# craston/object_detection_cib

Hardware: AMD Instinct MI355X
Metric: images/sec YOLOv5s 640px train (higher is better)
Workload: dtype bf16; 1 GPU; yv5s coco-zipf-like synthetic, 640px, bf16 storage/fp32 accumulate, batch 64/GPU, fwd+assign+loss+bwd+SGD, targets 4-30 boxes/img; global_batch=64, parallelism=dp1, launch=hipGraph replay, collectives=none, launcher=none, attempt=0

## Files before the change

### object_detection_cib_amd/csrc/conv_igemm.hip

```cpp
#include "kodhip_common.h"
#include <stdlib.h>
#include <type_traits>

extern "C" const char* kodhip_last_error(void);

namespace {

enum { MODE_RAW = 0, MODE_PLAIN = 1, MODE_HEAD = 2, MODE_PLAIN_BN = 3, MODE_FUSED = 4, MODE_FUSED_ACT = 5 };

constexpr bool mode_is_fused(int mode) { return mode == MODE_FUSED || mode == MODE_FUSED_ACT; }

constexpr int MAX_SEG = 3;

struct ConvArgs {
  const bf16_t* x;
  const bf16_t* w;
  bf16_t* y;
  float* stats;
  const float* bias;
  float* head_out;
  int B, Hs, Ws, ldx, xcoff, Cin;
  int cin_step;
  int Ho, Wo, M;
  int N, K, Kp;
  int KH, KW;
  int mul_h, mul_w, add_h, add_w, tap_sign, sh_shift, sw_shift;
  int ldy, ycoff, accumulate;
  float* y32;
  int f32_mode;
  int out_mul, out_off_y, out_off_x, out_H, out_W;
  int d2s_C;
  int d2s_skip;
  int head_A, head_P, head_nc;
  uint32_t magic_hp;
  uint32_t magic_cin, magic_kw;
  int tiles_m, tiles_n, groups_m, stats_slots;
  float rcp_hwo, rcp_wo;
  uint32_t x_bytes, w_bytes;
  const bf16_t* x2;
  const bf16_t* w2;
  int nk1;
  int wide_px;
  int pointwise;
  int nseg, slot_base, slot_used;
  int seg_begin[MAX_SEG], seg_end[MAX_SEG], seg_ldr[MAX_SEG], seg_C[MAX_SEG];
  const bf16_t* seg_raw[MAX_SEG];
  const float* seg_aff[MAX_SEG];
  float* seg_part[MAX_SEG];
  const float* scale;
  const float* shift;
  const bf16_t* residual;
  int ldr, rcoff;
  int act;
  float slope;
};

template <int ACT>
__device__ __forceinline__ bf16x4 fused_quad(const f32x16& acc, int g, const f32x4& sc, const f32x4& sh, float slope) {
  bf16x4 v;
#pragma unroll
  for (int e = 0; e < 4; ++e) v[e] = (bf16_t)kod_act<ACT>(__builtin_fmaf(acc[g * 4 + e], sc[e], sh[e]), slope);
  return v;
}

__device__ __forceinline__ void fast_divmod(int n, int d, float rcp, int& q, int& r) {
  q = (int)((float)n * rcp);
  r = n - q * d;
  while (r < 0) { --q; r += d; }
  while (r >= d) { ++q; r -= d; }
}

constexpr int BK = 32;

template <int N>
__device__ __forceinline__ void wait_vm_imm() { asm volatile("s_waitcnt vmcnt(%0)" ::"n"(N) : "memory"); }

template <int BM, int BN, int WAVES_M, int WAVES_N, int MODE, bool FAST, bool ROW3 = false, bool F32ACC = false, bool STEM = false>
__device__ __forceinline__ void conv_igemm_body(const ConvArgs& a, const int bid) {
  constexpr int NT = 64 * WAVES_M * WAVES_N;
  constexpr int NW = NT / 64;
  static_assert(FAST || (BM == 128 && NT == 256), "register-staged path is written for 128-row tiles / 4 waves");
  constexpr int LDS_ROW = FAST ? BK : BK + 8;
  constexpr int WM = BM / WAVES_M;
  constexpr int WN = BN / WAVES_N;
  constexpr int TM = WM / 32;
  constexpr int TN = WN / 32;
  constexpr int B_CHUNKS = BN * 4;
  constexpr int B_PER_THREAD = (B_CHUNKS + NT - 1) / NT;
  static_assert(!ROW3 || (FAST && BM == 128), "ROW3 is a FAST-path form for 128-pixel tiles");
  constexpr int A3_ROWS = BM + 16;
  static_assert(!STEM || (FAST && BM == 128 && !ROW3 && (MODE == MODE_RAW || mode_is_fused(MODE))), "STEM is a forward FAST-path form for 128-pixel tiles");
  constexpr int AS_ROWS = BM + 64;
  constexpr int STAGE_ELEMS = STEM ? AS_ROWS * 8 + BN * LDS_ROW : (ROW3 ? (A3_ROWS + 3 * BN) * LDS_ROW : (BM + BN) * LDS_ROW);
  constexpr int CS_ROW = BN + 8;
  constexpr int NST = (FAST && BM == 256 && !ROW3) ? 3 : 2;
  constexpr int LDS_ELEMS = (NST * STAGE_ELEMS > BM * CS_ROW) ? NST * STAGE_ELEMS : BM * CS_ROW;
  __shared__ __attribute__((aligned(16))) bf16_t lds[LDS_ELEMS];
  float* sred = reinterpret_cast<float*>(lds);

  const int tid = threadIdx.x;
  const int lane = tid & 63;
  const int wave = tid >> 6;
  const int wm = wave / WAVES_N;
  const int wn = wave % WAVES_N;

  const int xcd = bid & 7;
  const int j = bid >> 3;
  const int nt = j % a.tiles_n;
  const int gm = (j / a.tiles_n) * 8 + xcd;
  if (gm >= a.groups_m) return;
  const int n0 = nt * BN;

  const int a_chunk = tid & 3;
  const int a_row = tid >> 2;
  const int HWs = a.Hs * a.Ws;
  const int HWo = a.Ho * a.Wo;

  float ssum[8], ssq[8];
#pragma unroll
  for (int i = 0; i < 8; ++i) ssum[i] = ssq[i] = 0.f;
  float bn_run = 0.f;

  int nk_steps = STEM ? a.KH : (ROW3 ? 3 * (a.cin_step / BK) : (a.nk1 ? 2 * a.nk1 : a.Kp / BK));
  if constexpr ((MODE == MODE_PLAIN || MODE == MODE_PLAIN_BN) && FAST && !ROW3 && !STEM) {
    if (a.d2s_skip && n0 + BN <= 2 * a.d2s_C) nk_steps >>= 1;
  }
  const int nk = nk_steps;
  __amdgpu_buffer_rsrc_t rs_x, rs_w, rs_x2, rs_w2;
  if constexpr (FAST) {
    rs_x = __builtin_amdgcn_make_buffer_rsrc((void*)a.x, 0, a.x_bytes, 0x00020000);
    rs_w = __builtin_amdgcn_make_buffer_rsrc((void*)a.w, 0, a.w_bytes, 0x00020000);
    rs_x2 = __builtin_amdgcn_make_buffer_rsrc((void*)(a.nk1 ? a.x2 : a.x), 0, a.x_bytes, 0x00020000);
    rs_w2 = __builtin_amdgcn_make_buffer_rsrc((void*)(a.nk1 ? a.w2 : a.w), 0, a.w_bytes, 0x00020000);
  }

  const int gq = gm >> 3, gk = (a.groups_m - xcd + 7) >> 3;
  int gbefore = 0;
  for (int i = 0; i < xcd; ++i) gbefore += (a.groups_m - i + 7) >> 3;
  const int band_begin = (int)((long)a.tiles_m * gbefore / a.groups_m);
  const int band_end = (int)((long)a.tiles_m * (gbefore + gk) / a.groups_m);
  for (int mt = band_begin + gq; mt < band_end; mt += gk) {
    const int m0 = mt * BM;
    int rbase[2], rby[2], rbx[2];
    bool rvalid[2];
    const bf16_t* rptr[2];
    uint32_t rmask[2];
    const bool linear_taps = (a.sh_shift | a.sw_shift) == 0;
#pragma unroll
    for (int r = 0; r < 2; ++r) {
      int m = m0 + a_row + r * 64;
      rvalid[r] = m < a.M;
      int mm = rvalid[r] ? m : 0;
      int b, rem, oy, ox;
      fast_divmod(mm, HWo, a.rcp_hwo, b, rem);
      fast_divmod(rem, a.Wo, a.rcp_wo, oy, ox);
      rbase[r] = b * HWs;
      rby[r] = oy * a.mul_h + a.add_h;
      rbx[r] = ox * a.mul_w + a.add_w;
      rptr[r] = a.x + ((long)(rbase[r] + rby[r] * a.Ws + rbx[r]) * a.ldx + a.xcoff);
      uint32_t xm = 0, mk = 0;
      for (int kw = 0; kw < a.KW; ++kw)
        if ((unsigned)(rbx[r] + a.tap_sign * kw) < (unsigned)a.Ws) xm |= 1u << kw;
      for (int kh = 0; kh < a.KH; ++kh)
        if ((unsigned)(rby[r] + a.tap_sign * kh) < (unsigned)a.Hs) mk |= xm << (kh * a.KW);
      rmask[r] = rvalid[r] ? mk : 0u;
    }
    const bf16_t* bptr[B_PER_THREAD];
#pragma unroll
    for (int q = 0; q < B_PER_THREAD; ++q) {
      int c = tid + q * NT;
      int n = n0 + (c >> 2);
      bptr[q] = (c < B_CHUNKS && n < a.N) ? a.w + (size_t)n * a.Kp + (c & 3) * 8 : nullptr;
    }

    constexpr int B_INSTR = BN / 16;
    constexpr int B_PER_WAVE = (B_INSTR + NW - 1) / NW;
    const int uwave = __builtin_amdgcn_readfirstlane(wave);
    constexpr int A_PER_WAVE = BM / (16 * NW);
    static_assert(!FAST || A_PER_WAVE * 16 * NW == BM, "pixel tile rows must divide over the waves' DMA instructions");
    uint32_t dvoff[A_PER_WAVE > 0 ? A_PER_WAVE : 1], dmask[A_PER_WAVE > 0 ? A_PER_WAVE : 1], dbvoff[B_PER_WAVE];
    int f_tap = 0, f_kh = 0, f_kw = 0, f_ci = 0;
    if constexpr (FAST) {
#pragma unroll
      for (int i = 0; i < ((ROW3 || STEM) ? 0 : A_PER_WAVE); ++i) {
        int row = (uwave * A_PER_WAVE + i) * 16 + (lane >> 2);
        int m = m0 + row;
        bool valid = m < a.M;
        int mm = valid ? m : 0;
        int chunk = (lane & 3) ^ ((row >> 2) & 3);
        if (a.pointwise) {
          dvoff[i] = (uint32_t)(((long)mm * a.ldx + a.xcoff + chunk * 8) * 2);
          dmask[i] = valid ? 1u : 0u;
          continue;
        }
        int b, rem, oy, ox;
        fast_divmod(mm, HWo, a.rcp_hwo, b, rem);
        fast_divmod(rem, a.Wo, a.rcp_wo, oy, ox);
        int by = oy * a.mul_h + a.add_h, bx = ox * a.mul_w + a.add_w;
        dvoff[i] = (uint32_t)(((long)(b * HWs + by * a.Ws + bx) * a.ldx + a.xcoff + chunk * 8) * 2);
        const int bxl = a.wide_px > 1 ? bx + (chunk * 8) / a.ldx : bx;
        uint32_t xm = 0, mk = 0;
        for (int kw = 0; kw < a.KW; ++kw)
          if ((unsigned)(bxl + a.tap_sign * kw) < (unsigned)a.Ws) xm |= 1u << kw;
        for (int kh = 0; kh < a.KH; ++kh)
          if ((unsigned)(by + a.tap_sign * kh) < (unsigned)a.Hs) mk |= xm << (kh * a.KW);
        dmask[i] = valid ? mk : 0u;
      }
#pragma unroll
      for (int q = 0; q < B_PER_WAVE; ++q) {
        int row = (uwave * B_PER_WAVE + q) * 16 + (lane >> 2);
        int n = n0 + row;
        int chunk = (lane & 3) ^ ((row >> 2) & 3);
        dbvoff[q] = (row < BN && n < a.N) ? (uint32_t)(((size_t)n * a.Kp + chunk * 8) * 2) : 0xFFFFFFF0u;
      }
    }
    auto dma_tile = [&](int kt, int buf) {
      const uint32_t soff = (uint32_t)((a.tap_sign * (f_kh * a.Ws + f_kw) * a.ldx + f_ci) * 2);
      char* As = reinterpret_cast<char*>(lds + buf * STAGE_ELEMS);
      char* Bs = As + BM * LDS_ROW * 2;
      const bool second = a.nk1 != 0 && kt >= a.nk1;
      const int kw_step = second ? kt - a.nk1 : kt;
#if defined(__HIP_DEVICE_COMPILE__) && !defined(KOD_ABL_NODMA)
      const __amdgpu_buffer_rsrc_t rx = second ? rs_x2 : rs_x, rw = second ? rs_w2 : rs_w;
#pragma unroll
      for (int i = 0; i < A_PER_WAVE; ++i) {
        uint32_t vo = ((dmask[i] >> f_tap) & 1u) ? dvoff[i] + soff : 0xFFFFFFF0u;
        __builtin_amdgcn_raw_ptr_buffer_load_lds(rx, (__attribute__((address_space(3))) void*)(As + (uwave * A_PER_WAVE + i) * 16 * 64),
                                                 16, vo, 0, 0, 0);
      }
// ... 539 lines not shown
          if constexpr (MODE == MODE_PLAIN || MODE == MODE_PLAIN_BN) {
            if (a.out_mul != 1)
              opix = (size_t)(uint32_t)((pb * a.out_H + poy * a.out_mul) * a.out_W + pox * a.out_mul + pix_off);
          }
          bf16_t* dst = a.y + opix * a.ldy + a.ycoff + nch;
          if constexpr (MODE == MODE_PLAIN || MODE == MODE_PLAIN_BN) {
            if (a.accumulate && (!F32ACC || a.f32_mode < 2)) {
              bf16x8 o = *reinterpret_cast<const bf16x8*>(dst);
#pragma unroll
              for (int e = 0; e < 8; ++e) v[e] = (bf16_t)((float)v[e] + (float)o[e]);
            }
            if constexpr (MODE == MODE_PLAIN_BN) {
              if (sg_raw) {
#ifdef KOD_ABL_NOBNLOAD
                bf16x8 yv = v;
#else
                bf16x8 yv = *reinterpret_cast<const bf16x8*>(sg_raw + opix * sg_ldr);
#endif
#pragma unroll
                for (int e = 0; e < 8; ++e) {
#ifdef KOD_ABL_NOBNMATH
                  ssum[e] += (float)v[e]; ssq[e] += (float)yv[e]; continue;
#endif
                  const float y = (float)yv[e];
                  const float z = __builtin_fmaf(y, sg_sc[e], sg_sh[e]);
                  const float r = kod_sigmoid_l2(KOD_NEG_LOG2E * z);
                  const float dz = kod_silu_bwd((float)v[e], z, r);
                  ssum[e] += dz;
                  ssq[e] = __builtin_fmaf(dz, y, ssq[e]);
                }
              }
            }
          } else if constexpr (mode_is_fused(MODE)) {
            if (a.residual) {
              const bf16x8 r = *reinterpret_cast<const bf16x8*>(a.residual + (size_t)m * a.ldr + a.rcoff + n);
#pragma unroll
              for (int e = 0; e < 8; ++e) v[e] = (bf16_t)((float)v[e] + (float)r[e]);
            }
          } else {
#pragma unroll
            for (int e = 0; e < 8; ++e) {
              float f = (float)v[e];
              ssum[e] += f;
              ssq[e] += f * f;
            }
          }
#ifdef KOD_ABL_NOSTORE
          if (v[0] == (bf16_t)12345.f)
#endif
          *reinterpret_cast<bf16x8*>(dst) = v;
        }
      }
      __syncthreads();
      if constexpr (MODE == MODE_PLAIN_BN) {
#pragma unroll
        for (int o = CPR; o < 64; o <<= 1)
#pragma unroll
          for (int e = 0; e < 8; ++e) {
            ssum[e] += __shfl_xor(ssum[e], o, 64);
            ssq[e] += __shfl_xor(ssq[e], o, 64);
          }
        if (lane < CPR) {
#pragma unroll
          for (int e = 0; e < 8; ++e) {
            sred[(wave * BN + lane * 8 + e) * 2 + 0] = ssum[e];
            sred[(wave * BN + lane * 8 + e) * 2 + 1] = ssq[e];
          }
        }
#pragma unroll
        for (int e = 0; e < 8; ++e) ssum[e] = ssq[e] = 0.f;
        __syncthreads();
        if (tid < BN * 2) {
          const int ch = tid >> 1, st = tid & 1;
#pragma unroll
          for (int w = 0; w < NW; ++w) bn_run += sred[(w * BN + ch) * 2 + st];
        }
        __syncthreads();
      }
    }
  }

  if constexpr (MODE == MODE_PLAIN_BN) {
    if (tid < BN * 2) {
      const int ch = tid >> 1, st = tid & 1;
      int nn = n0 + ch, sbase = a.slot_base;
      if (a.d2s_C != 0) {
        const int cls = nn / a.d2s_C;
        nn -= cls * a.d2s_C; sbase = cls * a.groups_m;
        if (cls > 3) nn = -1;
      }
#pragma unroll
      for (int sgi = 0; sgi < MAX_SEG; ++sgi)
        if (sgi < a.nseg && nn >= a.seg_begin[sgi] && nn < a.seg_end[sgi]) {
          float* slot = a.seg_part[sgi] + ((size_t)st * a.seg_C[sgi] + (nn - a.seg_begin[sgi])) * a.stats_slots;
          slot[sbase + gm] = bn_run;
          for (int t = sbase + gm + a.slot_used; t < a.stats_slots; t += a.slot_used) slot[t] = 0.f;
        }
    }
  }
  if constexpr (MODE == MODE_RAW) {
    constexpr int CPR = BN / 8;
#pragma unroll
    for (int o = CPR; o < 64; o <<= 1)
#pragma unroll
      for (int e = 0; e < 8; ++e) {
        ssum[e] += __shfl_xor(ssum[e], o, 64);
        ssq[e] += __shfl_xor(ssq[e], o, 64);
      }
    if (lane < CPR) {
#pragma unroll
      for (int e = 0; e < 8; ++e) {
        sred[(wave * BN + lane * 8 + e) * 2 + 0] = ssum[e];
        sred[(wave * BN + lane * 8 + e) * 2 + 1] = ssq[e];
      }
    }
    __syncthreads();
    if (tid < BN * 2) {
      int ch = tid >> 1, st = tid & 1;
      float s = 0.f;
#pragma unroll
      for (int w = 0; w < NW; ++w) s += sred[(w * BN + ch) * 2 + st];
      int nn = n0 + ch;
      if (nn < a.N) {
        float* slot = a.stats + ((size_t)st * a.N + nn) * a.stats_slots;
        slot[gm] = s;
        for (int t = gm + a.groups_m; t < a.stats_slots; t += a.groups_m) slot[t] = 0.f;
      }
    }
  }
}

template <int BM, int BN, int WAVES_M, int WAVES_N, int MODE, bool FAST, bool F32ACC = false>
__global__ __launch_bounds__(64 * WAVES_M * WAVES_N, (MODE == 2  ? 2 : (FAST ? 4 : 3)))
void conv_igemm_kernel(ConvArgs a) {
  conv_igemm_body<BM, BN, WAVES_M, WAVES_N, MODE, FAST, false, F32ACC>(a, blockIdx.x);
}

template <int BN, int WAVES_M, int WAVES_N, int MODE, bool F32ACC = false>
__global__ __launch_bounds__(64 * WAVES_M * WAVES_N, (BN == 128 ? 2 : (BN == 64 ? 3 : 4)))
void conv_igemm_row3_kernel(ConvArgs a) {
  conv_igemm_body<128, BN, WAVES_M, WAVES_N, MODE, true, true, F32ACC>(a, blockIdx.x);
}

template <int BN, int WAVES_M, int WAVES_N, int MODE = MODE_RAW>
__global__ __launch_bounds__(64 * WAVES_M * WAVES_N, 4)
void conv_igemm_stem_kernel(ConvArgs a) {
  conv_igemm_body<128, BN, WAVES_M, WAVES_N, MODE, true, false, false, true>(a, blockIdx.x);
}

template <int MODE>
__device__ __forceinline__ void conv_stem_fwd_body(const ConvArgs& a) {
  constexpr bool FUSED = mode_is_fused(MODE);
  constexpr int BM = 128, BN = 32, NWV = 4;
  constexpr int PR = 192;
  constexpr int KHM = 6;
  constexpr int W_BYTES = KHM * BN * 64;
  constexpr int P_BYTES = KHM * PR * 16;
  constexpr int CS_ROW = BN + 8;
  __shared__ __attribute__((aligned(1024))) unsigned char lds[W_BYTES + 2 * P_BYTES];
  float* sred = reinterpret_cast<float*>(lds + W_BYTES);

  const int tid = threadIdx.x, lane = tid & 63;
  const int wave = __builtin_amdgcn_readfirstlane(tid >> 6);
  const int fr = lane & 31, fh = lane >> 5;
  const int HWo = a.Ho * a.Wo;
  const int grid = gridDim.x, blk = blockIdx.x;

#if defined(__HIP_DEVICE_COMPILE__)
  __amdgpu_buffer_rsrc_t rs_x = __builtin_amdgcn_make_buffer_rsrc((void*)a.x, 0, a.x_bytes, 0x00020000);
  __amdgpu_buffer_rsrc_t rs_w = __builtin_amdgcn_make_buffer_rsrc((void*)a.w, 0, a.w_bytes, 0x00020000);
#endif
#pragma unroll
  for (int i = 0; i < 3; ++i) {
    const int t = wave + NWV * i;
    const int kh = t >> 1, row = (t & 1) * 16 + (lane >> 2);
    const int chunk = (lane & 3) ^ ((row >> 2) & 3);
    const uint32_t vo = row < a.N ? (uint32_t)(((size_t)row * a.Kp + kh * 32 + chunk * 8) * 2) : 0xFFFFFFF0u;
#if defined(__HIP_DEVICE_COMPILE__)
    __builtin_amdgcn_raw_ptr_buffer_load_lds(rs_w, (__attribute__((address_space(3))) void*)(lds + t * 1024), 16, vo, 0, 0, 0);
#else
    (void)vo;
#endif
  }
  auto stage_tile = [&](int mt, int buf) {
    const int m0 = mt * BM;
    unsigned char* P = lds + W_BYTES + buf * P_BYTES;
#pragma unroll
    for (int i = 0; i < 5; ++i) {
      const int t = wave + NWV * i;
      if (t >= 18) continue;
      const int kh = t / 3, part = t - kh * 3;
      const int r = part * 64 + lane;
      const long q = (long)m0 - 1 + r;
      bool ok = r < BM + 3 && q >= 0 && q < a.M;
      int b, rem, oy, ox;
      fast_divmod(ok ? (int)q : 0, HWo, a.rcp_hwo, b, rem);
      fast_divmod(rem, a.Wo, a.rcp_wo, oy, ox);
      const int iy = oy * a.mul_h + a.add_h + kh;
      ok = ok && (unsigned)iy < (unsigned)a.Hs;
      const uint32_t vo = ok ? (uint32_t)(((long)(b * a.Hs + iy) * a.Ws + ox) * 16) : 0xFFFFFFF0u;
#if defined(__HIP_DEVICE_COMPILE__)
      __builtin_amdgcn_raw_ptr_buffer_load_lds(rs_x, (__attribute__((address_space(3))) void*)(P + t * 1024), 16, vo, 0, 0, 0);
#else
      (void)vo; (void)P;
#endif
    }
  };

  float ssum[8], ssq[8];
#pragma unroll
  for (int e = 0; e < 8; ++e) ssum[e] = ssq[e] = 0.f;

  const int my_p = wave < 2 ? 5 : 4;
  int buf = 0;
  const int xcd = blk & 7, bq = blk >> 3, bk = (grid - xcd + 7) >> 3;
  int bbefore = 0;
  for (int i = 0; i < xcd; ++i) bbefore += (grid - i + 7) >> 3;
  const int band_end = (int)((long)a.tiles_m * (bbefore + bk) / grid);
  const int mt0 = (int)((long)a.tiles_m * bbefore / grid) + bq;
  if (mt0 < band_end) stage_tile(mt0, 0);
  for (int mt = mt0; mt < band_end; mt += bk) {
    const int m0 = mt * BM;
    const bool more = mt + bk < band_end;
    if (more) stage_tile(mt + bk, buf ^ 1);
    if (more) { if (my_p == 5) wait_vm_imm<5>(); else wait_vm_imm<4>(); }
    else asm volatile("s_waitcnt vmcnt(0)" ::: "memory");
    __builtin_amdgcn_s_barrier();

    int pb, prem, poy, pox;
    const int pm = m0 + wave * 32 + fr;
    fast_divmod(pm < a.M ? pm : 0, HWo, a.rcp_hwo, pb, prem);
    fast_divmod(prem, a.Wo, a.rcp_wo, poy, pox);
    const bool ok0 = pox != 0, ok2 = pox != a.Wo - 1;

    f32x16 acc;
#pragma unroll
    for (int e = 0; e < 16; ++e) acc[e] = 0.f;
    const bf16_t* Wl = reinterpret_cast<const bf16_t*>(lds);
    const bf16_t* Pl = reinterpret_cast<const bf16_t*>(lds + W_BYTES + buf * P_BYTES);
#pragma unroll
    for (int kh = 0; kh < KHM; ++kh)
#pragma unroll
      for (int ks = 0; ks < 2; ++ks) {
        const int ch = (ks * 2 + fh) ^ ((fr >> 2) & 3);
        const bf16x8 wf = *reinterpret_cast<const bf16x8*>(Wl + (kh * BN + fr) * 32 + ch * 8);
        bf16x8 xf = *reinterpret_cast<const bf16x8*>(Pl + (kh * PR + wave * 32 + fr + ks * 2 + fh) * 8);
        if (ks == 0 && fh == 0 && !ok0) xf = bf16x8{};
        if (ks == 1 && fh == 0 && !ok2) xf = bf16x8{};
        acc = __builtin_amdgcn_mfma_f32_32x32x16_bf16(wf, xf, acc, 0, 0, 0);
      }
    __builtin_amdgcn_s_barrier();

    bf16_t* Cs = reinterpret_cast<bf16_t*>(lds + W_BYTES + buf * P_BYTES);
    if constexpr (FUSED) {
      auto stage = [&](auto actc) {
        constexpr int ACT = decltype(actc)::value;
#pragma unroll
        for (int g = 0; g < 4; ++g) {
          const int col = 8 * g + 4 * fh;
          f32x4 sc = {0.f, 0.f, 0.f, 0.f}, sh = {0.f, 0.f, 0.f, 0.f};
          if (col < a.N) {
            sc = *reinterpret_cast<const f32x4*>(a.scale + col);
            sh = *reinterpret_cast<const f32x4*>(a.shift + col);
          }
          *reinterpret_cast<bf16x4*>(Cs + (wave * 32 + fr) * CS_ROW + col) = fused_quad<ACT>(acc, g, sc, sh, a.slope);
        }
      };
      if constexpr (MODE == MODE_FUSED) stage(std::integral_constant<int, ACT_SILU>{});
      else kod_with_act<false>(a.act, stage);
    } else {
#pragma unroll
    for (int g = 0; g < 4; ++g) {
      bf16x4 v;
#pragma unroll
      for (int e = 0; e < 4; ++e) v[e] = (bf16_t)acc[g * 4 + e];
      *reinterpret_cast<bf16x4*>(Cs + (wave * 32 + fr) * CS_ROW + 8 * g + 4 * fh) = v;
    }
    }
    __syncthreads();
    const int c = tid & 3, r0 = tid >> 2;
    const bool col_ok = c * 8 < a.N;
#pragma unroll
    for (int p = 0; p < 2; ++p) {
      const int row = r0 + p * 64;
      const int m = m0 + row;
      if (m < a.M && col_ok) {
        bf16x8 v = *reinterpret_cast<const bf16x8*>(Cs + row * CS_ROW + c * 8);
        if constexpr (FUSED) {
          if (a.residual) {
            const bf16x8 r = *reinterpret_cast<const bf16x8*>(a.residual + (size_t)m * a.ldr + a.rcoff + c * 8);
#pragma unroll
            for (int e = 0; e < 8; ++e) v[e] = (bf16_t)((float)v[e] + (float)r[e]);
          }
        } else {
#pragma unroll
          for (int e = 0; e < 8; ++e) {
            const float f = (float)v[e];
            ssum[e] += f;
            ssq[e] += f * f;
          }
        }
        *reinterpret_cast<bf16x8*>(a.y + (size_t)m * a.ldy + a.ycoff + c * 8) = v;
      }
    }
    __syncthreads();
    buf ^= 1;
  }

  if constexpr (FUSED) return;
#pragma unroll
  for (int o = 4; o < 64; o <<= 1)
#pragma unroll
    for (int e = 0; e < 8; ++e) {
      ssum[e] += __shfl_xor(ssum[e], o, 64);
      ssq[e] += __shfl_xor(ssq[e], o, 64);
    }
  if (lane < 4) {
#pragma unroll
    for (int e = 0; e < 8; ++e) {
      sred[(wave * BN + lane * 8 + e) * 2 + 0] = ssum[e];
      sred[(wave * BN + lane * 8 + e) * 2 + 1] = ssq[e];
    }
  }
  __syncthreads();
  if (tid < BN * 2) {
    const int ch = tid >> 1, st = tid & 1;
    float sacc = 0.f;
#pragma unroll
    for (int w = 0; w < NWV; ++w) sacc += sred[(w * BN + ch) * 2 + st];
    if (ch < a.N) {
      float* slot = a.stats + ((size_t)st * a.N + ch) * a.stats_slots;
      slot[blk] = sacc;
      for (int t = blk + grid; t < a.stats_slots; t += grid) slot[t] = 0.f;
    }
  }
}

__global__ __launch_bounds__(256, 3) void conv_stem_fwd_kernel(ConvArgs a) { conv_stem_fwd_body<MODE_RAW>(a); }

template <int MODE>
__global__ __launch_bounds__(256, 3) void conv_stem_fwd_fused_kernel(ConvArgs a) { conv_stem_fwd_body<MODE>(a); }

struct ConvArgs4 { ConvArgs c[4]; int per_class; };

template <int BM, int BN, int WAVES_M, int WAVES_N, int MODE, bool FAST, bool F32ACC = false>
__global__ __launch_bounds__(64 * WAVES_M * WAVES_N, (MODE == 2  ? 2 : (FAST ? 4 : 3)))
void conv_igemm_x4_kernel(ConvArgs4 p) {
  const int bid = blockIdx.x;
  const int q = bid / p.per_class;
  const int cls = q == 0 ? 3 : (q == 3 ? 0 : q);
  conv_igemm_body<BM, BN, WAVES_M, WAVES_N, MODE, FAST, false, F32ACC>(p.c[cls], bid - q * p.per_class);
}


struct ConvKnobs {
  int force_bn, force_bm;
  int row3;
  int s2_fold_maxc;
  bool no_fast;
  bool s2_separate;
  bool no_bnred;
};
const ConvKnobs& conv_knobs() {
  static const ConvKnobs k = [] {
    auto num = [](const char* e, int dflt) { return e ? atoi(e) : dflt; };
    ConvKnobs v;
    v.force_bn = num(getenv("KODHIP_FORCE_BN"), 0);
    v.force_bm = num(getenv("KODHIP_FORCE_BM"), 0);
    v.row3 = num(getenv("KODHIP_ROW3"), 2);
    v.s2_fold_maxc = num(getenv("KODHIP_S2_FOLD_MAXC"), 64);
    v.no_fast = getenv("KODHIP_NO_FAST") != nullptr;
    v.s2_separate = getenv("KODHIP_S2_SEPARATE") != nullptr;
    v.no_bnred = getenv("KODHIP_NO_BNRED") != nullptr;
    return v;
  }();
  return k;
}

enum ConvForm { CONV_FAST, CONV_REG, CONV_ROW3, CONV_STEM_BODY, CONV_STEM, CONV_X4 };
struct ConvPlan {
  ConvForm form;
  bool fast;
  int bm, bn, waves_m, waves_n;
  int tiles_m, tiles_n, groups_m;
  int per_class, grid, block;
  int pointwise;
  uint32_t x_bytes, w_bytes[4];
  int bnred_slots;
};

long x_extent(const ConvArgs& a) { return (long)a.B * a.Hs * a.Ws * a.ldx * 2; }
long w_extent(const ConvArgs& a) { return (long)a.N * a.Kp * 2; }

bool fast_eligible(const ConvArgs& a) {
  return (a.cin_step % 32 == 0) && (a.sh_shift | a.sw_shift) == 0 && a.K == a.Kp && x_extent(a) < (1l << 32) - 64 &&
         w_extent(a) < (1l << 32) - 64 && !conv_knobs().no_fast;
}

int slots_for(int bm, int bn, bool fast) {
  if (bm == 256) return 512;
  if (fast) return 1024;
  return bn == 128 ? 1024 : (bn == 64 ? 1280 : 1536);
}

constexpr int MAX_STATS_SLOTS = 1024;
int stats_slots(long M) {
  long tiles_m = (M + 127) / 128;
  return tiles_m < MAX_STATS_SLOTS ? (int)tiles_m : MAX_STATS_SLOTS;
}

int widest_bn(int N) { return N > 64 ? 128 : (N > 32 ? 64 : 32); }

bool takes_256(long M, int N, int K, bool fast) {
  const int force_bm = conv_knobs().force_bm;
  return fast && widest_bn(N) >= 64 && M >= 256 * 64 && (force_bm ? force_bm == 256 : K >= 512);
}

void make_plan(ConvPlan& p, long M, int N, int K, bool fast, bool row3 = false) {
  const int force_bn = conv_knobs().force_bn;
  const int widest = widest_bn(N);
  const int bm = !row3 && takes_256(M, N, K, fast) ? 256 : 128;
  double best_cost = 1e30;
  for (int bn = widest; bn >= 32 && bn >= widest / 2; bn >>= 1) {
    if (bm == 256 && bn != widest) continue;
    if (force_bn && force_bn <= widest && bn != force_bn) continue;
    long tiles_m = (M + bm - 1) / bm, tiles_n = (N + bn - 1) / bn;
    int slots = slots_for(bm, bn, fast);
    if (row3) slots = bn == 128 ? 512 : (bn == 64 ? 768 : 1024);
    long rounds = (tiles_m * tiles_n + slots - 1) / slots;
    double cost = (double)rounds * (bm + bn);
    if (cost < best_cost * 0.97) {
      best_cost = cost;
      int target = slots / (int)tiles_n;
      if (target < 8) target = 8;
      if (target > MAX_STATS_SLOTS) target = MAX_STATS_SLOTS;
      p.bm = bm; p.bn = bn; p.tiles_m = (int)tiles_m; p.tiles_n = (int)tiles_n;
      p.groups_m = tiles_m < target ? (int)tiles_m : target;
      p.per_class = p.grid = cdiv(p.groups_m, 8) * 8 * (int)tiles_n;
    }
  }
  p.waves_m = p.bm == 256 || p.bn == 32 ? 4 : 2; p.waves_n = p.bn == 32 ? 1 : 2;
  p.block = 64 * p.waves_m * p.waves_n;
}

ConvPlan conv_plan(const ConvArgs& a, int mode) {
  ConvPlan p = {};
  p.fast = fast_eligible(a);
  const int K = a.nk1 ? 2 * a.K : a.K;
  const int row3_mode = conv_knobs().row3;
  const bool row3 = p.fast && row3_mode && a.KH == 3 && a.KW == 3 && a.mul_h == 1 && a.mul_w == 1 && a.Ho == a.Hs && a.Wo == a.Ws &&
                    a.add_h == -a.tap_sign && a.add_w == -a.tap_sign && a.wide_px == 1 && a.nk1 == 0 && a.d2s_C == 0 &&
                    a.out_mul == 1 && a.head_A == 0 && !(row3_mode == 1 && takes_256(a.M, a.N, K, p.fast));
  make_plan(p, a.M, a.N, K, p.fast, row3);
  p.form = row3 ? CONV_ROW3 : (p.fast ? CONV_FAST : CONV_REG);
  p.x_bytes = (uint32_t)x_extent(a); p.w_bytes[0] = (uint32_t)w_extent(a);
  p.pointwise = (p.fast && a.KH == 1 && a.KW == 1 && a.mul_h == 1 && a.mul_w == 1 && a.add_h == 0 && a.add_w == 0 &&
                 a.Ho == a.Hs && a.Wo == a.Ws && a.wide_px == 1 && (a.sh_shift | a.sw_shift) == 0) ? 1 : 0;
  p.bnred_slots = p.fast ? (a.d2s_C ? 4 : 1) * p.groups_m : 0;
  if ((mode == MODE_RAW || mode_is_fused(mode)) && p.fast && !row3 && a.wide_px == 4 && a.KW == 1 && a.mul_w == 1 && a.add_w == -1 &&
      a.ldx == 8 && a.xcoff == 0 && p.bm == 128 && (p.bn == 32 || p.bn == 64) && (long)a.M + 256 < (1l << 31)) {
// ... 402 lines not shown
```

Measured before the change: 5574 images/sec.

## Triple-buffer stem conv input tiles and keep weights and BN params in registers

Reworks the stem forward conv loop to prefetch two tiles ahead over three LDS buffers instead of double buffering, and shrinks each patch buffer to the rows actually needed. Per-tile pixel coordinates now advance incrementally rather than through repeated divmods. Weights and fused scale/shift are loaded into registers once, and LDS reads and writes use inline asm with explicit lgkm waits so fragment loads overlap the MFMAs. This adds LDS footprint and register pressure and relies on hand-counted vmcnt/lgkmcnt waits, which can break if the compiler reorders memory operations.

```diff
diff --git a/object_detection_cib_amd/csrc/conv_igemm.hip b/object_detection_cib_amd/csrc/conv_igemm.hip
--- a/object_detection_cib_amd/csrc/conv_igemm.hip
+++ b/object_detection_cib_amd/csrc/conv_igemm.hip
@@ -75,6 +75,18 @@
 template <int N>
 __device__ __forceinline__ void wait_vm_imm() { asm volatile("s_waitcnt vmcnt(%0)" ::"n"(N) : "memory"); }
 
+template <int N>
+__device__ __forceinline__ void wait_lgkm_imm() { asm volatile("s_waitcnt lgkmcnt(%0)" ::"n"(N) : "memory"); }
+template <int OFF>
+__device__ __forceinline__ void lds_read_b128(u32x4& d, uint32_t addr) {
+  asm volatile("ds_read_b128 %0, %1 offset:%2" : "=v"(d) : "v"(addr), "n"(OFF) : "memory");
+}
+template <int OFF>
+__device__ __forceinline__ void lds_write_b64(uint32_t addr, s16x4 v) {
+  asm volatile("ds_write_b64 %0, %1 offset:%2" ::"v"(addr), "v"(v), "n"(OFF) : "memory");
+}
+__device__ __forceinline__ void reg_tie(u32x4& a, u32x4& b) { asm volatile("" : "+v"(a), "+v"(b)); }
+
 template <int BM, int BN, int WAVES_M, int WAVES_N, int MODE, bool FAST, bool ROW3 = false, bool F32ACC = false, bool STEM = false>
 __device__ __forceinline__ void conv_igemm_body(const ConvArgs& a, const int bid) {
   constexpr int NT = 64 * WAVES_M * WAVES_N;
@@ -920,12 +932,19 @@
 __device__ __forceinline__ void conv_stem_fwd_body(const ConvArgs& a) {
   constexpr bool FUSED = mode_is_fused(MODE);
   constexpr int BM = 128, BN = 32, NWV = 4;
-  constexpr int PR = 192;
+  constexpr int DEPTH = 2;
+  constexpr int NBUF = DEPTH + 1;
+  constexpr int PR = BM + 3;
   constexpr int KHM = 6;
+  constexpr int SLOTS = KHM * PR;
+  constexpr int NI = (SLOTS + 63) / 64;
+  constexpr int NJ = (NI + NWV - 1) / NWV;
   constexpr int W_BYTES = KHM * BN * 64;
-  constexpr int P_BYTES = KHM * PR * 16;
+  constexpr int P_BYTES = NI * 1024;
   constexpr int CS_ROW = BN + 8;
-  __shared__ __attribute__((aligned(1024))) unsigned char lds[W_BYTES + 2 * P_BYTES];
+  static_assert(DEPTH == 2, "the waits below are written for two tiles ahead");
+  static_assert(BM * CS_ROW * 2 <= P_BYTES, "the store staging overlays one tile buffer");
+  __shared__ __attribute__((aligned(1024))) unsigned char lds[W_BYTES + NBUF * P_BYTES];
   float* sred = reinterpret_cast<float*>(lds + W_BYTES);
 
   const int tid = threadIdx.x, lane = tid & 63;
@@ -950,110 +969,190 @@
     (void)vo;
 #endif
   }
-  auto stage_tile = [&](int mt, int buf) {
-    const int m0 = mt * BM;
-    unsigned char* P = lds + W_BYTES + buf * P_BYTES;
-#pragma unroll
-    for (int i = 0; i < 5; ++i) {
-      const int t = wave + NWV * i;
-      if (t >= 18) continue;
-      const int kh = t / 3, part = t - kh * 3;
-      const int r = part * 64 + lane;
-      const long q = (long)m0 - 1 + r;
-      bool ok = r < BM + 3 && q >= 0 && q < a.M;
-      int b, rem, oy, ox;
-      fast_divmod(ok ? (int)q : 0, HWo, a.rcp_hwo, b, rem);
-      fast_divmod(rem, a.Wo, a.rcp_wo, oy, ox);
-      const int iy = oy * a.mul_h + a.add_h + kh;
-      ok = ok && (unsigned)iy < (unsigned)a.Hs;
-      const uint32_t vo = ok ? (uint32_t)(((long)(b * a.Hs + iy) * a.Ws + ox) * 16) : 0xFFFFFFF0u;
-#if defined(__HIP_DEVICE_COMPILE__)
-      __builtin_amdgcn_raw_ptr_buffer_load_lds(rs_x, (__attribute__((address_space(3))) void*)(P + t * 1024), 16, vo, 0, 0, 0);
-#else
-      (void)vo; (void)P;
-#endif
-    }
-  };
-
-  float ssum[8], ssq[8];
-#pragma unroll
-  for (int e = 0; e < 8; ++e) ssum[e] = ssq[e] = 0.f;
-
-  const int my_p = wave < 2 ? 5 : 4;
-  int buf = 0;
   const int xcd = blk & 7, bq = blk >> 3, bk = (grid - xcd + 7) >> 3;
   int bbefore = 0;
   for (int i = 0; i < xcd; ++i) bbefore += (grid - i + 7) >> 3;
   const int band_end = (int)((long)a.tiles_m * (bbefore + bk) / grid);
   const int mt0 = (int)((long)a.tiles_m * bbefore / grid) + bq;
-  if (mt0 < band_end) stage_tile(mt0, 0);
-  for (int mt = mt0; mt < band_end; mt += bk) {
-    const int m0 = mt * BM;
-    const bool more = mt + bk < band_end;
-    if (more) stage_tile(mt + bk, buf ^ 1);
-    if (more) { if (my_p == 5) wait_vm_imm<5>(); else wait_vm_imm<4>(); }
-    else asm volatile("s_waitcnt vmcnt(0)" ::: "memory");
+  const int ntile = mt0 < band_end ? (band_end - mt0 + bk - 1) / bk : 0;
+
+  int dB, dY, dX, drem;
+  fast_divmod(bk * BM, HWo, a.rcp_hwo, dB, drem);
+  fast_divmod(drem, a.Wo, a.rcp_wo, dY, dX);
+  dB = __builtin_amdgcn_readfirstlane(dB); dY = __builtin_amdgcn_readfirstlane(dY); dX = __builtin_amdgcn_readfirstlane(dX);
+
+  int sb[NJ], soy[NJ], sox[NJ], skh[NJ];
+#pragma unroll
+  for (int j = 0; j < NJ; ++j) {
+    const int L = (wave + NWV * j) * 64 + lane;
+    const int kh = L / PR, r = L - kh * PR;
+    skh[j] = L < SLOTS ? kh + a.add_h : -(1 << 30);
+    int rem;
+    fast_divmod(mt0 * BM + r, HWo, a.rcp_hwo, sb[j], rem);
+    fast_divmod(rem, a.Wo, a.rcp_wo, soy[j], sox[j]);
+    sox[j] -= 1;
+    if (sox[j] < 0) { sox[j] += a.Wo; soy[j] -= 1; }
+    if (soy[j] < 0) { soy[j] += a.Ho; sb[j] -= 1; }
+  }
+  auto stage_next = [&](int buf) {
+    unsigned char* P = lds + W_BYTES + buf * P_BYTES;
+#pragma unroll
+    for (int j = 0; j < NJ; ++j) {
+      const int i = wave + NWV * j;
+      if (i >= NI) continue;
+      const int iy = soy[j] * a.mul_h + skh[j];
+      const bool ok = (unsigned)sb[j] < (unsigned)a.B && (unsigned)iy < (unsigned)a.Hs;
+      const uint32_t vo = ok ? (uint32_t)((sb[j] * a.Hs + iy) * a.Ws + sox[j]) * 16u : 0xFFFFFFF0u;
+#if defined(__HIP_DEVICE_COMPILE__)
+      __builtin_amdgcn_raw_ptr_buffer_load_lds(rs_x, (__attribute__((address_space(3))) void*)(P + i * 1024), 16, vo, 0, 0, 0);
+#else
+      (void)vo; (void)P;
+#endif
+      sox[j] += dX;
+      const int cx = sox[j] >= a.Wo;
+      sox[j] -= cx ? a.Wo : 0;
+      soy[j] += dY + cx;
+      const int cy = soy[j] >= a.Ho;
+      soy[j] -= cy ? a.Ho : 0;
+      sb[j] += dB + cy;
+    }
+  };
+  auto wait_landed = [&](int younger) {
+    if (younger <= 0) asm volatile("s_waitcnt vmcnt(0)" ::: "memory");
+    else if (wave < NI - NWV * (NJ - 1)) wait_vm_imm<NJ>();
+    else wait_vm_imm<NJ - 1>();
+  };
+  auto lds_barrier = [&]() {
+    wait_lgkm_imm<0>();
     __builtin_amdgcn_s_barrier();
-
-    int pb, prem, poy, pox;
-    const int pm = m0 + wave * 32 + fr;
-    fast_divmod(pm < a.M ? pm : 0, HWo, a.rcp_hwo, pb, prem);
+  };
+
+  float ssum[8], ssq[8];
+#pragma unroll
+  for (int e = 0; e < 8; ++e) ssum[e] = ssq[e] = 0.f;
+
+  f32x4 fsc[4], fsh[4];
+#pragma unroll
+  for (int g = 0; g < 4; ++g) {
+    fsc[g] = f32x4{0.f, 0.f, 0.f, 0.f}; fsh[g] = f32x4{0.f, 0.f, 0.f, 0.f};
+    if constexpr (FUSED) {
+      const int col = 8 * g + 4 * fh;
+      if (col < a.N) {
+        fsc[g] = *reinterpret_cast<const f32x4*>(a.scale + col);
+        fsh[g] = *reinterpret_cast<const f32x4*>(a.shift + col);
+      }
+      asm volatile("" : "+v"(fsc[g]), "+v"(fsh[g]));
+    }
+  }
+
+  const uint32_t lds_base = (uint32_t)(uintptr_t)(__attribute__((address_space(3))) unsigned char*)lds;
+  const int ch0 = fh ^ ((fr >> 2) & 3);
+  const uint32_t wa0 = lds_base + (uint32_t)(fr * 64 + ch0 * 16), wa1 = lds_base + (uint32_t)(fr * 64 + (ch0 ^ 2) * 16);
+  const uint32_t xa = lds_base + (uint32_t)(W_BYTES + (wave * 32 + fr + fh) * 16);
+  const uint32_t csw = lds_base + (uint32_t)(W_BYTES + ((wave * 32 + fr) * CS_ROW + 4 * fh) * 2);
+  const int c = tid & 3, r0 = tid >> 2;
+  const uint32_t csr = lds_base + (uint32_t)(W_BYTES + (r0 * CS_ROW + c * 8) * 2);
+  const bool col_ok = c * 8 < a.N;
+
+  int pox;
+  {
+    int pb, prem, poy;
+    fast_divmod(mt0 * BM + wave * 32 + fr, HWo, a.rcp_hwo, pb, prem);
     fast_divmod(prem, a.Wo, a.rcp_wo, poy, pox);
+  }
+
+#pragma unroll
+  for (int d = 0; d < DEPTH; ++d)
+    if (d < ntile) stage_next(d);
+  wait_landed(ntile > 1 ? 1 : 0);
+  lds_barrier();
+  u32x4 wq[KHM][2];
+#pragma unroll
+  for (int kh = 0; kh < KHM; ++kh) {
+    lds_read_b128<0>(wq[kh][0], wa0 + (uint32_t)(kh * BN * 64));
+    lds_read_b128<0>(wq[kh][1], wa1 + (uint32_t)(kh * BN * 64));
+  }
+  wait_lgkm_imm<0>();
+#pragma unroll
+  for (int kh = 0; kh < KHM; ++kh) reg_tie(wq[kh][0], wq[kh][1]);
+  int cur = 0, nxt = DEPTH % NBUF;
+  for (int k = 0; k < ntile; ++k) {
+    const int m0 = (mt0 + k * bk) * BM;
+    lds_barrier();
+    if (k + DEPTH < ntile) stage_next(nxt);
+
     const bool ok0 = pox != 0, ok2 = pox != a.Wo - 1;
-
+    const uint32_t xb = xa + (uint32_t)(cur * P_BYTES);
     f32x16 acc;
 #pragma unroll
     for (int e = 0; e < 16; ++e) acc[e] = 0.f;
-    const bf16_t* Wl = reinterpret_cast<const bf16_t*>(lds);
-    const bf16_t* Pl = reinterpret_cast<const bf16_t*>(lds + W_BYTES + buf * P_BYTES);
-#pragma unroll
-    for (int kh = 0; kh < KHM; ++kh)
+    u32x4 xq[2][2];
+    auto frag = [&](auto khc) {
+      constexpr int kh = decltype(khc)::value;
+      lds_read_b128<kh * PR * 16>(xq[kh & 1][0], xb);
+      lds_read_b128<kh * PR * 16 + 32>(xq[kh & 1][1], xb);
+    };
+    auto mult = [&](auto khc) {
+      constexpr int kh = decltype(khc)::value;
+      if constexpr (kh + 1 < KHM) {
+        frag(std::integral_constant<int, kh + 1>{});
+        wait_lgkm_imm<2>();
+      } else {
+        wait_lgkm_imm<0>();
+      }
+      reg_tie(xq[kh & 1][0], xq[kh & 1][1]);
 #pragma unroll
       for (int ks = 0; ks < 2; ++ks) {
-        const int ch = (ks * 2 + fh) ^ ((fr >> 2) & 3);
-        const bf16x8 wf = *reinterpret_cast<const bf16x8*>(Wl + (kh * BN + fr) * 32 + ch * 8);
-        bf16x8 xf = *reinterpret_cast<const bf16x8*>(Pl + (kh * PR + wave * 32 + fr + ks * 2 + fh) * 8);
+        const bf16x8 wf = __builtin_bit_cast(bf16x8, wq[kh][ks]);
+        bf16x8 xf = __builtin_bit_cast(bf16x8, xq[kh & 1][ks]);
         if (ks == 0 && fh == 0 && !ok0) xf = bf16x8{};
         if (ks == 1 && fh == 0 && !ok2) xf = bf16x8{};
         acc = __builtin_amdgcn_mfma_f32_32x32x16_bf16(wf, xf, acc, 0, 0, 0);
       }
-    __builtin_amdgcn_s_barrier();
-
-    bf16_t* Cs = reinterpret_cast<bf16_t*>(lds + W_BYTES + buf * P_BYTES);
+    };
+    frag(std::integral_constant<int, 0>{});
+    mult(std::integral_constant<int, 0>{}); mult(std::integral_constant<int, 1>{}); mult(std::integral_constant<int, 2>{});
+    mult(std::integral_constant<int, 3>{}); mult(std::integral_constant<int, 4>{}); mult(std::integral_constant<int, 5>{});
+    lds_barrier();
+
+    const uint32_t cw = csw + (uint32_t)(cur * P_BYTES), cr = csr + (uint32_t)(cur * P_BYTES);
+    auto put = [&](auto gc, bf16x4 v) {
+      constexpr int g = decltype(gc)::value;
+      lds_write_b64<g * 16>(cw, __builtin_bit_cast(s16x4, v));
+    };
     if constexpr (FUSED) {
       auto stage = [&](auto actc) {
         constexpr int ACT = decltype(actc)::value;
-#pragma unroll
-        for (int g = 0; g < 4; ++g) {
-          const int col = 8 * g + 4 * fh;
-          f32x4 sc = {0.f, 0.f, 0.f, 0.f}, sh = {0.f, 0.f, 0.f, 0.f};
-          if (col < a.N) {
-            sc = *reinterpret_cast<const f32x4*>(a.scale + col);
-            sh = *reinterpret_cast<const f32x4*>(a.shift + col);
-          }
-          *reinterpret_cast<bf16x4*>(Cs + (wave * 32 + fr) * CS_ROW + col) = fused_quad<ACT>(acc, g, sc, sh, a.slope);
-        }
+        put(std::integral_constant<int, 0>{}, fused_quad<ACT>(acc, 0, fsc[0], fsh[0], a.slope));
+        put(std::integral_constant<int, 1>{}, fused_quad<ACT>(acc, 1, fsc[1], fsh[1], a.slope));
+        put(std::integral_constant<int, 2>{}, fused_quad<ACT>(acc, 2, fsc[2], fsh[2], a.slope));
+        put(std::integral_constant<int, 3>{}, fused_quad<ACT>(acc, 3, fsc[3], fsh[3], a.slope));
       };
       if constexpr (MODE == MODE_FUSED) stage(std::integral_constant<int, ACT_SILU>{});
       else kod_with_act<false>(a.act, stage);
     } else {
-#pragma unroll
-    for (int g = 0; g < 4; ++g) {
-      bf16x4 v;
-#pragma unroll
-      for (int e = 0; e < 4; ++e) v[e] = (bf16_t)acc[g * 4 + e];
-      *reinterpret_cast<bf16x4*>(Cs + (wave * 32 + fr) * CS_ROW + 8 * g + 4 * fh) = v;
-    }
-    }
-    __syncthreads();
-    const int c = tid & 3, r0 = tid >> 2;
-    const bool col_ok = c * 8 < a.N;
+      auto raw_quad = [&](int g) {
+        bf16x4 v;
+#pragma unroll
+        for (int e = 0; e < 4; ++e) v[e] = (bf16_t)acc[g * 4 + e];
+        return v;
+      };
+      put(std::integral_constant<int, 0>{}, raw_quad(0)); put(std::integral_constant<int, 1>{}, raw_quad(1));
+      put(std::integral_constant<int, 2>{}, raw_quad(2)); put(std::integral_constant<int, 3>{}, raw_quad(3));
+    }
+    lds_barrier();
+    if (k + 1 < ntile) wait_landed(k + 2 < ntile ? 1 : 0);
+    u32x4 cq[2];
+    lds_read_b128<0>(cq[0], cr);
+    lds_read_b128<64 * CS_ROW * 2>(cq[1], cr);
+    wait_lgkm_imm<0>();
+    reg_tie(cq[0], cq[1]);
 #pragma unroll
     for (int p = 0; p < 2; ++p) {
       const int row = r0 + p * 64;
       const int m = m0 + row;
       if (m < a.M && col_ok) {
-        bf16x8 v = *reinterpret_cast<const bf16x8*>(Cs + row * CS_ROW + c * 8);
+        bf16x8 v = __builtin_bit_cast(bf16x8, cq[p]);
         if constexpr (FUSED) {
           if (a.residual) {
             const bf16x8 r = *reinterpret_cast<const bf16x8*>(a.residual + (size_t)m * a.ldr + a.rcoff + c * 8);
@@ -1071,9 +1170,12 @@
         *reinterpret_cast<bf16x8*>(a.y + (size_t)m * a.ldy + a.ycoff + c * 8) = v;
       }
     }
-    __syncthreads();
-    buf ^= 1;
-  }
+    pox += dX;
+    pox -= pox >= a.Wo ? a.Wo : 0;
+    cur = cur + 1 == NBUF ? 0 : cur + 1;
+    nxt = nxt + 1 == NBUF ? 0 : nxt + 1;
+  }
+  lds_barrier();
 
   if constexpr (FUSED) return;
 #pragma unroll
```

New measurement: 5586 images/sec, median of 6. No clear change (+0.2%).
